# LMNS3d/SOFTX_2020_200

Hardware: AMD Instinct MI355X
Metric: nonlinear iters/sec (3D cavity Q2 128^3 BDF2) (higher is better)
Workload: dtype f64; 1 GPU; 3D lid-driven cavity Q2-Q2 128^3 transient BDF2 (BASELINE configs[2]); n_dofs=67898372, n_cells=2097152, parallelism=single

## Files before the change

include/gls_native.h:

```cpp
#ifndef GLS_NATIVE_H
#define GLS_NATIVE_H

#include <stddef.h>
#include <stdint.h>

#ifdef __cplusplus
extern "C" {
#endif

#define GLS_OK 0
#define GLS_EINVAL -1
#define GLS_EHIP -2
#define GLS_ENOMEM -3
#define GLS_ENOCONV -4
#define GLS_EIO -5
#define GLS_ECOMM -6
#define GLS_ENOTFOUND -7

enum gls_scheme {
  GLS_STEADY = 0, GLS_BDF1, GLS_BDF2, GLS_BDF3, GLS_SDIRK2, GLS_SDIRK2_1, GLS_SDIRK2_2,
  GLS_SDIRK3, GLS_SDIRK3_1, GLS_SDIRK3_2, GLS_SDIRK3_3
};

const char *gls_last_error(void);
// ... 76 lines not shown
  double coarse_omega;
  int coarse_direct;
  int mixed_precision;
  const int *level_sweeps;
  int smoother;
  int smoother_operator;
} gls_mg_params;
int gls_mg_attach(gls_ctx *ctx, const gls_mg_params *prm);
int gls_mg_attach_transfers(gls_ctx *ctx, const gls_mg_params *prm, const int64_t *const *p_off,
                            const int32_t *const *p_col, const double *const *p_w, const int64_t *const *inject);
int gls_mg_attach_replica(gls_ctx *ctx, const gls_mg_params *prm, gls_ctx *replica, const int64_t *p_off,
                          const int32_t *p_col, const double *p_w, const int64_t *inject);
int gls_apply_preconditioner(gls_ctx *ctx, const double *v, double *z);
int gls_mg_smoother_apply(gls_ctx *ctx, const double *v, double *y);
int gls_mg_transfer(gls_ctx *ctx, int level, int direction, const double *in, double *out);
int gls_set_lattice(gls_ctx *ctx, int n1d, const int64_t *local_to_global);
int gls_mg_detach(gls_ctx *ctx);
int gls_mg_set_coarse_replica(gls_ctx *ctx, gls_ctx *replica, int64_t n_local, const int64_t *local_to_replica);
#define GLS_ILU_MAX_FILL 10
int gls_ilu_attach(gls_ctx *ctx, int fill, double athresh, double rthresh);
int gls_ilu_detach(gls_ctx *ctx);
#define GLS_ILU_ORDER_CM 0
#define GLS_ILU_ORDER_MULTICOLOR 1
int gls_ilu_set_options(gls_ctx *ctx, int ordering, int64_t block_dofs);
int gls_ilu_info(const gls_ctx *ctx, int64_t *nnz, int *n_probes);
int gls_ilu_matrix(gls_ctx *ctx, int32_t *rowp, int32_t *col, double *val);
int gls_ilu_factors(gls_ctx *ctx, int32_t *perm, int32_t *rowp, int32_t *col, double *val);
int gls_iluk_pattern(int64_t n, const int32_t *rowp, const int32_t *col, int fill, int32_t *out_rowp,
                     int32_t *out_col, int32_t *out_level, int64_t capacity, int64_t *out_nnz);
int gls_cuthill_mckee(int64_t n_nodes, const int64_t *adj_off, const int64_t *adj, const int64_t *dof_off,
// ... 225 lines not shown
```

softx_2020_200_amd/csrc/gls_api.cpp:

```cpp
#include <hip/hip_runtime.h>

#include <algorithm>
#include <array>
#include <chrono>
#include <cmath>
#include <cstdlib>
#include <cstdarg>
#include <cstdio>
#include <cstring>
#include <map>
#include <array>
#include <memory>
#include <string>
#include <vector>
#include <set>
#include <thread>

#include <rocblas/rocblas.h>
#include <rocsolver/rocsolver.h>
#include <rocsparse/rocsparse.h>
#include <rccl/rccl.h>

#include "../../include/gls_native.h"
#include "gls_common.hpp"
// ... 387 lines not shown
    DevBuf<int32_t> map;
  } lat;
  struct MG {
    bool on = false;
    bool boxed = false;
    std::vector<gls_ctx *> lev;
    std::vector<std::array<int, 3>> dims;
    int k = 2, pre = 2, post = 2, csweeps = 30;
    std::vector<int> lpre, lpost;
    double omega = 0.6, comega = 0.6;
    std::vector<std::unique_ptr<DevBuf<double>>> bufs;
    struct Taps {
      DevBuf<int32_t> pi[3], ri[3], pc[3], rc[3];
      DevBuf<double> pw[3], rw[3];
      bool two_pass = false;
    };
    std::vector<std::unique_ptr<Taps>> taps;
    bool csr = false;
    bool ilu_smooth = false;
    struct Csr {
      DevBuf<int64_t> poff, roff;
      DevBuf<int32_t> pcol, rcol, inj;
      DevBuf<double> pw, rw;
      int64_t nf = 0, nc = 0;
      int plane = 1, rlane = 1;
    };
    std::vector<std::unique_ptr<Csr>> xfer;
    std::vector<gls_ctx *> ilu_levels;
    DevBuf<double> xwork;
    bool direct = false, direct_ok = false;
// ... 2124 lines not shown
    const auto &T = *mg.taps[(size_t)l];
    const int32_t *ti[3] = {T.pi[0].p, T.pi[1].p, T.pi[2].p}, *tc[3] = {T.pc[0].p, T.pc[1].p, T.pc[2].p};
    const double *tw[3] = {T.pw[0].p, T.pw[1].p, T.pw[2].p};
    if (T.two_pass)
      HIP_TRY(gls::mg_transfer_2pass(xb, mg_box_target(c, l, y), mg.dims[l + 1].data(), mg.dims[l].data(), 0, ti, tw,
                                     tc, mg.xwork.p, s, add ? 1 : 0));
    else if (add)
      return set_err(GLS_EINVAL, "mg_prolong: accumulate needs the two-pass transfer");
    else
      HIP_TRY(gls::mg_transfer3d(xb, mg_box_target(c, l, y), mg.dims[l + 1].data(), mg.dims[l].data(), ti, tw, tc, s));
  }
  GLS_TRY(mg_from_box(c, l, y));
  return GLS_OK;
}

bool coarse_graph_eligible(gls_ctx *c, gls_ctx *g, const double *b, const double *x) {
  const int l = (int)c->mg.lev.size() - 1;
  return !c->mg.cgraph_failed && !c->mg.boxed && !g->dist.on && !g->hang.on && g->use_brick && g->use_qdata &&
         brick_slab(g) && gls::brick_fused_jacobi_supported(g->k) && g->stream == c->stream &&
         b == mgbuf(c, l, MB_B) && x == mgbuf(c, l, MB_X) && std::getenv("GLS_MG_NO_FUSE") == nullptr &&
         std::getenv("GLS_MG_GRAPH") != nullptr;
}
}
static std::vector<unsigned char> coarse_graph_key(gls_ctx *g, const double *b, const double *x, const double *y,
                                                   int pre, double om) {
  const gls::OpParams P = make_params(g);
  const void *ptrs[7] = {b, x, y, g->diag.p, g->qdata.p, g->qdata32.p, brick_slab(g)};
  const int64_t ints[4] = {pre, g->n_dofs, (int64_t)g->smooth_f32, (int64_t)slab_f32()};
  std::vector<unsigned char> k(sizeof(P) + sizeof(ptrs) + sizeof(ints) + sizeof(om));
  unsigned char *o = k.data();
// ... 209 lines not shown
    }
  }
  const bool first_fused = pre == 1 && l < L - 1 && first_sweep_fusable(g);
  double *zs = mg.ilu_smooth && g->ilu.on && !g->ilu.probe_only ? mgbuf(c, l, MB_BOX) : nullptr;
  if (pre > 0 && !first_fused && zs) {
    GLS_TRY(ensure_ilu(g));
    GLS_TRY(apply_ilu(g, b, x));
    for (int it = 1; it < pre; ++it) GLS_TRY(smoother_sweep(g, x, b, y, om, zs));
  } else if (pre > 0 && !first_fused) {
    HIP_TRY(gls::mg_jacobi_update(x, b, nullptr, d, om, n, 1, s));
    for (int it = 1; it < pre; ++it) GLS_TRY(smoother_sweep(g, x, b, y, om));
  } else if (pre == 0) {
    HIP_TRY(gls::vec_fill(x, n, 0.0, s));
  }
  if (l == L - 1) return GLS_OK;
  if (first_fused) {
    GLS_TRY(jacobian_apply_f32(g, x, y, b, om, g->smooth_oseen));
  } else if (pre > 0) {
    GLS_TRY(smoother_apply(g, x, y, b));
  } else {
    HIP_TRY(gls::vec_copy(y, b, n, s));
  }
  gls_ctx *h = mg.lev[l + 1];
  double *bc = mgbuf(c, l + 1, MB_B), *xc = mgbuf(c, l + 1, MB_X);
  GLS_TRY(mg_restrict(c, l, y, bc));
  HIP_TRY(gls::vec_set_indexed(bc, h->con_dofs.p, nullptr, (int64_t)h->con_dofs.n, s));
  GLS_TRY(mg_vcycle(c, l + 1, bc, xc));
  if (mg_prolong_add_ok(c, l)) {
    GLS_TRY(mg_prolong(c, l, xc, x, true));
  } else {
    GLS_TRY(mg_prolong(c, l, xc, y));
    HIP_TRY(gls::vec_set_indexed(y, g->con_dofs.p, nullptr, (int64_t)g->con_dofs.n, s));
    HIP_TRY(gls::vec_axpy(x, 1.0, y, n, s));
  }
  for (int it = 0; it < mg.lpost[(size_t)l]; ++it) GLS_TRY(smoother_sweep(g, x, b, y, mg.omega, zs));
  return GLS_OK;
}

#define RS_TRY(x)                                                                        \
  do {                                                                                   \
    const rocsparse_status rs_ = (x);                                                    \
// ... 211 lines not shown
  if (c->mg.on) GLS_TRY(mg_prepare(c));
  GLS_TRY(ensure_ilu(c));
  return apply_prec(c, v, z);
}

int gls_mg_transfer(gls_ctx *c, int level, int direction, const double *in, double *out) {
  GLS_TRY(check_ctx(c));
  auto &mg = c->mg;
  if (!mg.on) return set_err(GLS_EINVAL, "gls_mg_transfer: no multigrid attached");
  if (level < 0 || level + 1 >= (int)mg.lev.size() || (direction != 0 && direction != 1) || !in || !out || in == out)
    return set_err(GLS_EINVAL, "gls_mg_transfer: bad level / direction / pointers");
  if (direction == 0) return mg_restrict(c, level, in, out);
  double *xc = mgbuf(c, level + 1, MB_X);
  HIP_TRY(gls::vec_copy(xc, in, mg.lev[(size_t)level + 1]->n_dofs, c->stream));
  return mg_prolong(c, level, xc, out);
}

namespace {
int build_face_neighbours(gls_ctx *c) {
  const int dim = c->dim, k = c->k, nv = gls::ipow(k + 1, dim);
  std::vector<int32_t> cn((size_t)c->n_cells * nv);
  if (!cn.empty() && hipMemcpy(cn.data(), c->cell_vnodes.p, cn.size() * sizeof(int32_t), hipMemcpyDeviceToHost) != hipSuccess)
    return set_err(GLS_EHIP, "cell map download failed");
  std::map<std::array<int32_t, 4>, std::pair<int, int>> open;
  std::vector<int32_t> nbr((size_t)c->n_cells * 2 * dim, -1);
  for (int cell = 0; cell < c->n_cells; ++cell)
    for (int d = 0; d < dim; ++d)
      for (int sd = 0; sd < 2; ++sd) {
        std::array<int32_t, 4> key = {-1, -1, -1, -1};
        int nk = 0;
// ... 353 lines not shown
      }
    } else {
      const int n = (int)std::lround(std::cbrt((double)g->n_vnodes));
      if ((int64_t)n * n * n != g->n_vnodes) return set_err(GLS_EINVAL, "mg level %d is not an n^3 lattice", l);
      if (l > 0 && mg.dims.back()[0] != 2 * n - 1) return set_err(GLS_EINVAL, "mg level %d not nested", l);
      dm = {n, n, n};
    }
    mg.lev.push_back(g);
    mg.dims.push_back(dm);
  }
  const int K = c->k;
  size_t xwork = 0;
  for (int l = 0; l + 1 < p->n_levels; ++l) {
    std::unique_ptr<gls_ctx::MG::Taps> T(new gls_ctx::MG::Taps);
    T->two_pass = true;
    xwork = std::max(xwork, (size_t)4 * mg.dims[l + 1][0] * mg.dims[l + 1][1] * mg.dims[l][2]);
    for (int a = 0; a < 3; ++a) {
      const int nf = mg.dims[l][a], nc = mg.dims[l + 1][a], ncc = (nf - 1) / (2 * K);
      std::vector<int32_t> pi((size_t)nf * 5, 0), ri((size_t)nc * 5, 0);
      std::vector<double> pw((size_t)nf * 5, 0.0), rw((size_t)nc * 5, 0.0);
      std::vector<int32_t> rn((size_t)nc, 0), pn((size_t)nf, 0);
      for (int i = 0; i < nf; ++i) {
        const double x = (double)i / (2.0 * K);
        const int cc = std::min((int)std::floor(x), ncc - 1);
        const double xi = x - cc;
        int np = 0;
        for (int q = 0; q <= K; ++q) {
          double L = 1.0;
          for (int b = 0; b <= K; ++b)
            if (b != q) L *= (xi * K - b) / (double)(q - b);
          if (L == 0.0) continue;
          const int j = cc * K + q;
          pi[(size_t)i * 5 + np] = j;
          pw[(size_t)i * 5 + np] = L;
          ++np;
          if (rn[(size_t)j] >= 5) return set_err(GLS_EINVAL, "mg: restriction stencil wider than 5");
          ri[(size_t)j * 5 + rn[(size_t)j]] = i;
          rw[(size_t)j * 5 + rn[(size_t)j]] = L;
          ++rn[(size_t)j];
        }
        pn[(size_t)i] = np;
      }
      if (a < 2)
        T->two_pass = T->two_pass && gls::mg_transfer_tile_fits(0, a, nf, pi.data(), pn.data()) &&
                      gls::mg_transfer_tile_fits(1, a, nc, ri.data(), rn.data());
      GLS_TRY(T->pi[a].upload(pi.data(), pi.size()));
      GLS_TRY(T->pw[a].upload(pw.data(), pw.size()));
      GLS_TRY(T->ri[a].upload(ri.data(), ri.size()));
      GLS_TRY(T->rw[a].upload(rw.data(), rw.size()));
      GLS_TRY(T->pc[a].upload(pn.data(), pn.size()));
      GLS_TRY(T->rc[a].upload(rn.data(), rn.size()));
    }
    mg.taps.push_back(std::move(T));
  }
  if (xwork) GLS_TRY(mg.xwork.alloc(xwork));
  return mg_attach_common(c, p);
// ... 1851 lines not shown
```

softx_2020_200_amd/csrc/gls_brick_kernels.hip:

```cpp
#include "gls_brick_common.hpp"
#include "gls_common.hpp"
#include "gls_launch.hpp"

#include <algorithm>
#include <cstdlib>
#include <type_traits>

#ifndef GLS_ABL
#define GLS_ABL 0
#endif
#ifndef GLS_ROWS_REG
#define GLS_ROWS_REG 1
#endif
#ifndef GLS_BRICK_WAVES_PER_EU
#define GLS_BRICK_WAVES_PER_EU 4
#endif
#ifndef GLS_BRICK_WPE_F32
#define GLS_BRICK_WPE_F32 6
#endif

#ifndef GLS_QD_LITE
#define GLS_QD_LITE 0
#endif

// ... 1206 lines not shown
    if (jb) hipLaunchKernelGGL((k_slab_sum_cube<float, true, KK>), g, b, 0, s, slabf, nb1, voff, y, vmask, jb, jd, jomega, rb, x0);  \
    else hipLaunchKernelGGL((k_slab_sum_cube<float, false, KK>), g, b, 0, s, slabf, nb1, voff, y, vmask, jb, jd, jomega, rb, x0);   \
  } else {                                                                                                                  \
    if (jb) hipLaunchKernelGGL((k_slab_sum_cube<double, true, KK>), g, b, 0, s, slab, nb1, voff, y, vmask, jb, jd, jomega, rb, x0); \
    else hipLaunchKernelGGL((k_slab_sum_cube<double, false, KK>), g, b, 0, s, slab, nb1, voff, y, vmask, jb, jd, jomega, rb, x0);  \
  }
  if (k == 1) {
    GLS_SLAB_CUBE(1)
  } else {
    GLS_SLAB_CUBE(2)
  }
#undef GLS_SLAB_CUBE
  return hipGetLastError();
}

bool brick_fused_jacobi_supported(int k) { return brick_impl(k) == 0 && (k == 1 || k == 2); }
#ifdef GLS_BRICK_COLORS_BUILD
bool brick_colors_supported(int k) { return brick_impl(k) == 0 && (k == 1 || k == 2); }
#else
bool brick_colors_supported(int) { return false; }
#endif
bool brick_subset_supported(int k) { return brick_impl(k) == 0 && (k == 1 || k == 2); }

size_t brick_qdata_size(int k, int n_cells) {
  if (brick_impl(k) == 1) return brick_wave_qdata_size(k, n_cells);
  return k == 1 ? brick_qdata_doubles<1>(n_cells) : (k == 2 ? brick_qdata_doubles<2>(n_cells) : 0);
}

hipError_t launch_brick_kernel(int k, int mode, const OpParams &P, const Tables1D &T, hipStream_t s) {
  if (mode == MODE_DIAG) return hipErrorNotSupported;
// ... 8 lines not shown
```

softx_2020_200_amd/csrc/gls_brick_pencil.hip:

```cpp
#include "gls_brick_common.hpp"
#include "gls_common.hpp"
#include "gls_launch.hpp"

#include <cstdlib>
#include <type_traits>

#ifndef GLS_PENCIL_WPE64
#define GLS_PENCIL_WPE64 2
#endif
#ifndef GLS_PENCIL_PIPE
#define GLS_PENCIL_PIPE 1
#endif
#ifndef GLS_PENCIL_NT
#define GLS_PENCIL_NT 0
#endif
#ifndef GLS_PENCIL_WPE32
#define GLS_PENCIL_WPE32 4
#endif

namespace gls {

template <typename Real, bool JV>
struct PencilCfg {
  static constexpr int K1 = 3, N3 = 27, BN = 5, BN3 = 125, BN3P = 128, NBND = 98;
// ... 17 lines not shown
  using C = PencilCfg<Real, JV>;
  return sizeof(Real) * ((size_t)C::BPG * pencil_fields(mode) * C::FB + (size_t)C::WAVES * C::CPW * C::CS +
                         (size_t)C::CPG * C::OC) +
         sizeof(int) * (size_t)C::BPG * C::BN3P;
}
template <typename Real>
size_t pencil_lds_bytes(int mode) {
  return mode == MODE_JVQ ? pencil_lds_bytes_t<Real, true>(mode) : pencil_lds_bytes_t<Real, false>(mode);
}

template <typename Real>
struct PencilTab {
  Real V[3][3], D[3][3], S[3][3], w[3], xi[3];
};

template <typename Real, int MODE, bool GEN, bool FOREST = false, bool OS = false>
__global__ void __launch_bounds__(256, (std::is_same<Real, float>::value ? GLS_PENCIL_WPE32 : GLS_PENCIL_WPE64))
    gls_pencil_kernel(const OpParams P, const PencilTab<Real> T) {
  static_assert(!OS || (MODE == MODE_JVQ && std::is_same<Real, float>::value), "Oseen operator: FP32 J.v only");
  using C = PencilCfg<Real, MODE == MODE_JVQ>;
  constexpr bool RL = MODE == MODE_RESLIN, RES = MODE == MODE_RESIDUAL || RL, LIN = MODE == MODE_LIN || RL;
  constexpr bool ST = RES || LIN;
  constexpr int BN = C::BN, BN3 = C::BN3, BN3P = C::BN3P, NF = pencil_fields(MODE);
  extern __shared__ __attribute__((aligned(16))) char smem_raw[];
  constexpr int FB = C::FB, SY = C::SY, SZ = C::SZ;
  Real *const sB = reinterpret_cast<Real *>(smem_raw);
  Real *const sS = sB + C::BPG * NF * FB;
  constexpr int CS = C::CS;
  Real *const sO = sS + C::WAVES * C::CPW * CS;
  int *const sNode = reinterpret_cast<int *>(sO + C::CPG * C::OC);
  __shared__ Real sRow[3 * 16];

  const int tid = threadIdx.x, lane = tid & 63, wave = tid >> 6;
  const int n_bricks = P.n_cells / 8;
// ... 249 lines not shown
          *reinterpret_cast<d2 *>(slo + si + 2) = d2{(double)s[2], (double)s[3]};
        }
      }
    }
  };

  auto write_ev = [&]() {
    for (int t = tid; t < nbg * 8 * 27; t += C::THREADS) {
      const int rb_ = t / 216, r = t - rb_ * 216, ci_ = r / 27, a = r - ci_ * 27;
      const Real *o = sO + (rb_ * 8 + ci_) * C::OC + a;
      double *e = P.ev + (cell0(brick_of(rb_)) + ci_) * 108;
      e[a * 3] = (double)o[0];
      e[a * 3 + 1] = (double)o[C::OF];
      e[a * 3 + 2] = (double)o[2 * C::OF];
      e[81 + a] = (double)o[3 * C::OF];
    }
  };

  if constexpr (ST) {
    Real uq[3][3], Ttq[3][3], pq[3], gp[3][3];
    {
      Real dz[3];
#pragma unroll
      for (int cc = 0; cc < 3; ++cc) {
        Real bb[3], hb[3];
        forward(cc, 0, bb, dz, dz, dz);
        forward(4 + cc, 0, hb, dz, dz, dz);
#pragma unroll
        for (int qz = 0; qz < 3; ++qz) {
          uq[cc][qz] = zval(bb, qz);
// ... 298 lines not shown
      const Real JxW = wxy * T.w[qz], jt = JxW * tauq[qz];
      const Real Tv = JxW * divv[qz];
      const Real Tx = jt * Sq[0][qz] * ihx, Ty = jt * Sq[1][qz] * ihy, Tz = jt * Sq[2][qz] * ihz;
#pragma unroll
      for (int az = 0; az < 3; ++az) {
        Z[0][az] += T.V[qz][az] * Tv + T.D[qz][az] * Tz;
        Z[1][az] += T.V[qz][az] * Tx;
        Z[2][az] += T.V[qz][az] * Ty;
      }
    }
    backward(3, Z);
  }
  }
  __syncthreads();

  if (P.ev) write_ev();
  else reduce_scatter(P.y, P.slab, true);
}


bool pencil_enabled() {
  const char *e = std::getenv("GLS_PENCIL");
  return !(e && std::atoi(e) == 0);
}

template <typename Real, int MODE, bool FB = false>
hipError_t launch_pencil_t(const OpParams &P, const Tables1D &T, hipStream_t s) {
  const bool gen = P.srf || (MODE != MODE_JVQ && P.force_q);
  const int n_items = ((std::is_same<Real, double>::value || P.brick_cell0) && P.subset) ? P.subset_n : P.n_cells / 8;
  if (n_items <= 0) return hipSuccess;
  const int n_groups = (n_items + 2) / 3;
  PencilTab<Real> tab;
// ... 18 lines not shown
    }
  }
  if (gen)
    hipLaunchKernelGGL((gls_pencil_kernel<Real, MODE, true, FB>), dim3((unsigned)n_groups), dim3(256),
                       pencil_lds_bytes<Real>(MODE), s, P, tab);
  else
    hipLaunchKernelGGL((gls_pencil_kernel<Real, MODE, false, FB>), dim3((unsigned)n_groups), dim3(256),
                       pencil_lds_bytes<Real>(MODE), s, P, tab);
  return hipGetLastError();
}
hipError_t launch_pencil_jv(const OpParams &P, const Tables1D &T, hipStream_t s, bool f32) {
  if (P.n_probe > 0 || P.bricks || !(f32 ? (P.slabf != nullptr || P.slab != nullptr) : P.slab != nullptr))
    return hipErrorNotSupported;
  return f32 ? launch_pencil_t<float, MODE_JVQ>(P, T, s) : launch_pencil_t<double, MODE_JVQ>(P, T, s);
}
hipError_t launch_pencil_residual(const OpParams &P, const Tables1D &T, hipStream_t s) {
  if (P.bricks || !P.slab || P.subset) return hipErrorNotSupported;
  return launch_pencil_t<double, MODE_RESIDUAL>(P, T, s);
}
hipError_t launch_pencil_reslin(const OpParams &P, const Tables1D &T, hipStream_t s) {
  if (P.bricks || P.subset || !P.qd || !P.y || !P.slab || !P.res_y || !P.res_slab) return hipErrorNotSupported;
  return launch_pencil_t<double, MODE_RESLIN>(P, T, s);
}
hipError_t launch_pencil_ev(int mode, const OpParams &P, const Tables1D &T, hipStream_t s, bool f32) {
  if ((!P.ev && mode != MODE_LIN) || P.y || !P.brick_cell0 || !P.subset || P.subset_n <= 0 || !P.qd || P.slab ||
      P.bricks || P.n_probe > 0 || P.rb || P.jx || P.jx0 || (f32 && (mode != MODE_JVQ || !P.qdf)))
    return hipErrorNotSupported;
  if (mode == MODE_JVQ && f32) return launch_pencil_t<float, MODE_JVQ, true>(P, T, s);
  if (mode == MODE_JVQ) return launch_pencil_t<double, MODE_JVQ>(P, T, s);
  if (mode == MODE_LIN) return launch_pencil_t<double, MODE_LIN>(P, T, s);
// ... 9 lines not shown
```

softx_2020_200_amd/csrc/gls_common.hpp:

```cpp
#pragma once
#include <hip/hip_runtime.h>

#include <cstdint>

namespace gls {

constexpr int kMaxNodes1D = 4;
constexpr int kMaxQ1D = 5;

constexpr int ipow(int b, int e) { return e == 0 ? 1 : b * ipow(b, e - 1); }

enum Mode { MODE_RESIDUAL = 0, MODE_JV = 1, MODE_DIAG = 2, MODE_LIN = 3, MODE_JVQ = 4,
            MODE_RESLIN = 5  };
constexpr int kQData = 16;

struct Tables1D {
  double V[kMaxQ1D][kMaxNodes1D];
  double D[kMaxQ1D][kMaxNodes1D];
  double S[kMaxQ1D][kMaxNodes1D];
  double Vp[kMaxQ1D][kMaxNodes1D];
  double Dp[kMaxQ1D][kMaxNodes1D];
  double w[kMaxQ1D];
  double xi[kMaxQ1D];
};
// ... 45 lines not shown
  const int32_t *bricks;
  const uint16_t *ncolor;
  double *acc;
  int n_colors;
  int color;
  int color_off[17];
  double nu;
  double alpha[4];
  double alpha_jac;
  double sdt2;
  int srf;
  double omega[3];
  int oseen;
  double *cq;
  int cq_mode;
};

}
```

softx_2020_200_amd/csrc/gls_launch.hpp:

```cpp
#pragma once
#include "gls_common.hpp"

namespace gls {

hipError_t gather_element_vectors(double *y, const double *ev, const int64_t *voff, const int64_t *vslot, int64_t nv,
                                  const int64_t *poff, const int64_t *pslot, int64_t np, int dim, hipStream_t s);
hipError_t launch_cell_kernel(int dim, int k, int kp, int nq1d, int mode, const OpParams &P, const Tables1D &T,
                              hipStream_t s);
bool cell_kernel_supported(int dim, int k, int kp, int nq1d);
hipError_t launch_cell_sf_jv(int dim, int k, int kp, int nq1d, const OpParams &P, const Tables1D &T, hipStream_t s);
bool cell_sf_enabled();
int cell_kernel_cells_per_block(int dim, int k, int nq1d, bool probe = false);
hipError_t launch_brick_kernel(int k, int mode, const OpParams &P, const Tables1D &T, hipStream_t s);
size_t brick_qdata_size(int k, int n_cells);
hipError_t launch_brick_jv_f32(int k, const OpParams &P, const Tables1D &T, hipStream_t s);
hipError_t vec_to_f32(const double *a, float *b, int64_t n, hipStream_t s);
hipError_t vec_from_f32(const float *a, double *b, int64_t n, hipStream_t s);
hipError_t launch_pencil_jv(const OpParams &P, const Tables1D &T, hipStream_t s, bool f32);
hipError_t launch_pencil_residual(const OpParams &P, const Tables1D &T, hipStream_t s);
hipError_t launch_pencil_lin(const OpParams &P, const Tables1D &T, hipStream_t s);
hipError_t launch_pencil_reslin(const OpParams &P, const Tables1D &T, hipStream_t s);
hipError_t launch_pencil_ev(int mode, const OpParams &P, const Tables1D &T, hipStream_t s, bool f32 = false);
bool pencil_enabled();
hipError_t launch_brick_wave(int k, int mode, const OpParams &P, const Tables1D &T, hipStream_t s);
hipError_t launch_brick_wave_jv_f32(int k, const OpParams &P, const Tables1D &T, hipStream_t s);
hipError_t launch_brick_wave_probe(int k, const OpParams &P, const Tables1D &T, int64_t j0, int nprobe, hipStream_t s);
size_t brick_wave_qdata_size(int k, int n_cells);

int brick_boundary_nodes(int k);
hipError_t brick_slab_sum(const double *slab, const int32_t *nodes, const int32_t *off, const int32_t *slots,
                          int64_t n_sum, int64_t n_vnodes, double *y, hipStream_t s);
hipError_t brick_slab_sum_ex(const double *slab, const float *slabf, const int32_t *nodes, const int32_t *off,
                             const int32_t *slots, int64_t n_sum, int64_t n_vnodes, double *y, const uint8_t *vmask,
                             const double *jb, const double *jd, double jomega, hipStream_t s,
                             const double *rb = nullptr);
hipError_t brick_slab_sum_cube(int k, int nb1, const double *slab, const float *slabf, int64_t n_vnodes, double *y,
                               const uint8_t *vmask, const double *jb, const double *jd, double jomega, hipStream_t s,
                               const double *rb = nullptr, double *x0 = nullptr);
bool brick_fused_jacobi_supported(int k);
bool brick_colors_supported(int k);
bool brick_subset_supported(int k);
hipError_t launch_brick_probe(int k, const OpParams &P, const Tables1D &T, int64_t j0, int nprobe, hipStream_t s);

hipError_t vec_fill(double *x, int64_t n, double a, hipStream_t s);
hipError_t vec_copy(double *y, const double *x, int64_t n, hipStream_t s);
hipError_t vec_axpy(double *y, double a, const double *x, int64_t n, hipStream_t s);
hipError_t vec_axpby(double *y, double a, const double *x, double b, int64_t n, hipStream_t s);
hipError_t vec_scale(double *x, double a, int64_t n, hipStream_t s);
hipError_t vec_div(double *y, const double *x, const double *d, int64_t n, hipStream_t s);
hipError_t vec_multidot(const double *A, int64_t lda, int nk, const double *w, int64_t n, double *out,
                        double *work, hipStream_t s);
hipError_t vec_multidot2(const double *A, int64_t lda, int nk, const double *w, int64_t n1, int64_t off2, int64_t n2,
                         double *out, double *work, hipStream_t s);
// ... 117 lines not shown
```

softx_2020_200_amd/native.py:

```python
from __future__ import annotations

import ctypes as C
import os

import numpy as np

HERE = os.path.dirname(os.path.abspath(__file__))
LIB_PATH = os.environ.get("GLS_NATIVE_LIB") or os.path.join(HERE, "libgls_native.so")

GLS_OK, GLS_EINVAL, GLS_EHIP, GLS_ENOMEM, GLS_ENOCONV, GLS_EIO, GLS_ECOMM = 0, -1, -2, -3, -4, -5, -6

SCHEMES = {
    "steady": 0, "bdf1": 1, "bdf2": 2, "bdf3": 3, "sdirk2": 4, "sdirk2_1": 5, "sdirk2_2": 6,
    "sdirk3": 7, "sdirk3_1": 8, "sdirk3_2": 9, "sdirk3_3": 10,
}

EXPORTS = [
    "gls_last_error", "gls_version", "gls_create", "gls_destroy", "gls_set_stream", "gls_n_dofs", "gls_set_force",
    "gls_set_viscosity", "gls_set_time", "gls_set_state", "gls_residual", "gls_jacobian_apply",
    "gls_jacobian_apply_f32",
    "gls_jacobian_diagonal", "gls_set_dirichlet", "gls_apply_dirichlet", "gls_solve_linear", "gls_newton_solve",
    "gls_bdf_coefficients", "gls_sdirk_coefficients", "gls_newton_selftest", "gls_mesh_hyper_cube_sizes",
    "gls_mesh_hyper_cube", "gls_timing_reset", "gls_timing_get", "gls_timing_enable", "gls_uses_brick_kernels",
    "gls_part_create", "gls_part_sizes", "gls_part_get", "gls_part_destroy", "gls_dist_attach", "gls_dist_import", "gls_rccl_unique_id", "gls_rccl_create", "gls_rccl_destroy", "gls_rccl_info", "gls_mg_smoother_apply", "gls_mg_attach_replica",
    "gls_dist_attach_rccl",
    "gls_mg_attach", "gls_mg_detach", "gls_mg_set_coarse_replica", "gls_residual_and_diagonal", "gls_octree_set_periodic", "gls_ilu_attach", "gls_ilu_detach", "gls_ilu_info", "gls_ilu_matrix", "gls_ilu_factors", "gls_ilu_set_options", "gls_iluk_pattern", "gls_cuthill_mckee", "gls_section_timing", "gls_section_get", "gls_dist_attach_dofs", "gls_dist_attach_dofs_rccl", "gls_gpart_create", "gls_gpart_sizes", "gls_gpart_get", "gls_gpart_map_dofs", "gls_gpart_destroy", "gls_dpart_create", "gls_set_lattice", "gls_apply_preconditioner", "gls_mg_transfer",
    "gls_prm_parse", "gls_prm_get", "gls_prm_n_entries", "gls_prm_entry", "gls_prm_destroy",
    "gls_expr_create", "gls_expr_n_components", "gls_expr_eval", "gls_expr_destroy",
    "gls_vtu_write", "gls_pvtu_write", "gls_pvd_write",
    "gls_set_hanging", "gls_mesh_refined_create", "gls_mesh_refined_destroy", "gls_octree_create", "gls_octree_destroy", "gls_octree_info",
    "gls_octree_cells", "gls_octree_adapt", "gls_octree_prepare", "gls_octree_mesh", "gls_octree_mesh_destroy", "gls_octree_transfer", "gls_octree_faces", "gls_kelly_estimate_faces",
    "gls_kelly_estimate", "gls_refine_fixed_number", "gls_mesh_refined_interpolate", "gls_refine_pd", "gls_refine_coarsen_pd",
    "gls_freeze_jacobian", "gls_skip_newton_selftest", "gls_quadrature_points",
    "gls_umesh_generate", "gls_umesh_read_gmsh", "gls_umesh_set_manifold", "gls_umesh_boundary_manifold",
    "gls_umesh_refine_global", "gls_umesh_info", "gls_umesh_destroy", "gls_umesh_fe_space", "gls_fe_space_destroy",
    "gls_fe_space_transfer", "gls_umesh_prepare", "gls_umesh_adapt", "gls_umesh_set_periodic", "gls_fe_space_kelly_faces",
    "gls_kelly_estimate_mapped", "gls_fe_space_boundary_normals", "gls_fe_space_boundary_normal_sets",
    "gls_octree_coarsen_to", "gls_octree_mg_transfer", "gls_mg_attach_transfers", "gls_umesh_coarsen_to",
    "gls_fe_space_mg_transfer", "gls_forest_bricks",
    "gls_fe_space_boundary_faces", "gls_boundary_plan_create", "gls_boundary_plan_destroy", "gls_boundary_loads",
]
# ... 119 lines not shown
    L.gls_mg_set_coarse_replica.argtypes = [vp, vp, i64, C.POINTER(i64)]
    L.gls_mg_attach_transfers.argtypes = [vp, C.POINTER(MGParams), C.POINTER(C.POINTER(i64)),
                                          C.POINTER(C.POINTER(C.c_int32)), C.POINTER(C.POINTER(C.c_double)),
                                          C.POINTER(C.POINTER(i64))]
    L.gls_octree_coarsen_to.argtypes = [vp, C.c_int, C.POINTER(vp)]
    L.gls_umesh_coarsen_to.argtypes = [vp, C.c_int, C.POINTER(vp)]
    L.gls_forest_bricks.argtypes = [vp]
    L.gls_fe_space_mg_transfer.argtypes = [C.POINTER(FESpace), C.POINTER(FESpace), C.POINTER(i64), vp, vp, vp, vp]
    L.gls_octree_mg_transfer.argtypes = [C.POINTER(RefinedMesh), C.POINTER(RefinedMesh), C.POINTER(i64), vp, vp, vp, vp]
    L.gls_set_lattice.argtypes = [vp, C.c_int, C.POINTER(i64)]
    L.gls_apply_preconditioner.argtypes = [vp, vp, vp]
    L.gls_mg_smoother_apply.argtypes = [vp, vp, vp]
    L.gls_mg_attach_replica.argtypes = [vp, C.POINTER(MGParams), vp, C.POINTER(C.c_int64), C.POINTER(C.c_int32),
                                        C.POINTER(C.c_double), C.POINTER(C.c_int64)]
    L.gls_mg_transfer.argtypes = [vp, C.c_int, C.c_int, vp, vp]
    P64 = C.POINTER(i64)
    L.gls_set_hanging.argtypes = [vp, i64, P64, P64, P64, d]
    L.gls_mesh_refined_create.argtypes = [C.c_int, C.c_int, C.c_int, C.c_int, C.c_double, C.c_double,
                                          C.POINTER(C.c_int32), C.POINTER(C.POINTER(RefinedMesh))]
    L.gls_mesh_refined_destroy.argtypes = [C.POINTER(RefinedMesh)]
    L.gls_kelly_estimate.argtypes = [vp, vp, C.c_int, vp]
    L.gls_refine_fixed_number.argtypes = [i64, C.POINTER(C.c_float), C.c_double, C.POINTER(C.c_int32)]
    L.gls_refine_pd.argtypes = [i64, C.POINTER(C.c_float), C.c_int, C.c_int, C.c_double, i64,
                                C.POINTER(C.c_int32), C.POINTER(C.c_double)]
    L.gls_mesh_refined_interpolate.argtypes = [C.POINTER(RefinedMesh), C.c_int, C.c_double, C.c_double,
                                               C.POINTER(C.c_double), C.POINTER(C.c_double)]
    L.gls_quadrature_points.argtypes = [vp, d]
    L.gls_umesh_generate.argtypes = [C.c_int, C.c_char_p, C.c_char_p, C.POINTER(vp)]
    L.gls_umesh_read_gmsh.argtypes = [C.c_int, C.c_char_p, C.POINTER(vp)]
    L.gls_umesh_set_manifold.argtypes = [vp, C.c_int, C.c_int, d, d]
# ... 612 lines not shown
        check(self.L.gls_boundary_plan_create(self.h, len(sl), int(faces["nqf"]), p32(f["cell"]), p32(sl), _dp(f["xi"]),
                                              _dp(f["jinv"]), _dp(f["normal"]), _dp(f["jxw"]), _dp(f["xq"]),
                                              int(n_slots), C.byref(plan)), "gls_boundary_plan_create")
        force, torque = np.zeros((int(n_slots), 3)), np.zeros((int(n_slots), 3))
        try:
            check(self.L.gls_boundary_loads(self.h, plan, _ptr(sol), float(viscosity), _dp(cor), _dp(force), _dp(torque)),
                  "gls_boundary_loads")
        finally:
            self.L.gls_boundary_plan_destroy(plan)
        return force, torque

    def mg_transfer(self, level, direction, v, out):
        check(self.L.gls_mg_transfer(self.h, int(level), int(direction), _ptr(v), _ptr(out)), "gls_mg_transfer")
        return out

    def set_lattice(self, n1d, local_to_global):
        l2g = np.ascontiguousarray(local_to_global, dtype=np.int64)
        check(self.L.gls_set_lattice(self.h, int(n1d), l2g.ctypes.data_as(C.POINTER(C.c_int64))), "gls_set_lattice")

    def detach_multigrid(self):
        check(self.L.gls_mg_detach(self.h), "gls_mg_detach")
        self._mg_levels = None

    def attach_ilu(self, athresh=1e-8, rthresh=1.0, fill=0, block_dofs=0, ordering="cm"):
        self.L.gls_ilu_set_options.argtypes = [C.c_void_p, C.c_int, C.c_int64]
        check(self.L.gls_ilu_set_options(self.h, {"cm": 0, "multicolor": 1}[ordering], int(block_dofs)),
              "gls_ilu_set_options")
        self.L.gls_ilu_attach.argtypes = [C.c_void_p, C.c_int, C.c_double, C.c_double]
        check(self.L.gls_ilu_attach(self.h, int(fill), float(athresh), float(rthresh)), "gls_ilu_attach")
        nnz, npr = C.c_int64(), C.c_int()
# ... 268 lines not shown
```

Baseline: 11.51 nonlinear_iters/s.

## Fuse multigrid residual computation with Q2 restriction inside the pencil operator kernel

Adds a restriction epilogue to the FP32 pencil J.v kernel. It computes the residual b - Av per brick in LDS, applies the 5-to-3 Q2 restriction stencil along each axis, and writes per-brick coarse contributions to the slab. A new cube-sum kernel then gathers these into the coarse right-hand side and applies Dirichlet masking. This replaces the separate smoother-apply, two-pass transfer and constrained-dof zeroing kernels, with the aim of cutting full fine-level vector round trips in each V-cycle. It only applies under many eligibility conditions (structured cube, Q2 weights, brick/slab path), and it adds LDS pressure and new code paths.

```diff
diff --git a/include/gls_native.h b/include/gls_native.h
--- a/include/gls_native.h
+++ b/include/gls_native.h
@@ -114,6 +114,7 @@
 int gls_apply_preconditioner(gls_ctx *ctx, const double *v, double *z);
 int gls_mg_smoother_apply(gls_ctx *ctx, const double *v, double *y);
 int gls_mg_transfer(gls_ctx *ctx, int level, int direction, const double *in, double *out);
+int gls_mg_residual_restrict(gls_ctx *ctx, int level, const double *x, const double *b, double *bc, int *fused);
 int gls_set_lattice(gls_ctx *ctx, int n1d, const int64_t *local_to_global);
 int gls_mg_detach(gls_ctx *ctx);
 int gls_mg_set_coarse_replica(gls_ctx *ctx, gls_ctx *replica, int64_t n_local, const int64_t *local_to_replica);
diff --git a/softx_2020_200_amd/csrc/gls_api.cpp b/softx_2020_200_amd/csrc/gls_api.cpp
--- a/softx_2020_200_amd/csrc/gls_api.cpp
+++ b/softx_2020_200_amd/csrc/gls_api.cpp
@@ -425,6 +425,7 @@
       DevBuf<int32_t> pi[3], ri[3], pc[3], rc[3];
       DevBuf<double> pw[3], rw[3];
       bool two_pass = false;
+      bool q2_brick = false;
     };
     std::vector<std::unique_ptr<Taps>> taps;
     bool csr = false;
@@ -2579,6 +2580,46 @@
   return GLS_OK;
 }
 
+bool mg_fused_restrict_ok(gls_ctx *c, int l) {
+  auto &mg = c->mg;
+  if (l < 0 || l + 1 >= (int)mg.lev.size() || mg.csr || mg.boxed || (size_t)l >= mg.taps.size()) return false;
+  const char *e = std::getenv("GLS_MG_FUSE_TRANSFER");
+  if ((e && std::atoi(e) == 0) || std::getenv("GLS_MG_NO_FUSE") != nullptr) return false;
+  gls_ctx *g = mg.lev[(size_t)l], *h = mg.lev[(size_t)l + 1];
+  const auto &T = *mg.taps[(size_t)l];
+  const int64_t nc1 = 2 * (int64_t)g->cube_nb1 + 1;
+  return T.two_pass && T.q2_brick && g->smooth_f32 && g->use_brick && g->use_qdata && !g->use_colors && !g->dist.on &&
+         !g->hang.on && !g->oct.on && g->k == 2 && g->cube_nb1 > 0 && g->cube_nb1 < 1024 && g->use_slab && !g->srf &&
+         gls::pencil_enabled() && gls::brick_fused_jacobi_supported(g->k) && !h->dist.on && !h->hang.on &&
+         h->n_vnodes == nc1 * nc1 * nc1 && g->stream == c->stream;
+}
+int mg_residual_restrict_fused(gls_ctx *c, int l, double *x, const double *b, double *bc, double first_omega = 0.0) {
+  gls_ctx *g = c->mg.lev[(size_t)l], *h = c->mg.lev[(size_t)l + 1];
+  if (!g->u) return set_err(GLS_EINVAL, "gls_set_state was not called");
+  GLS_TRY(ensure_diag(g));
+  GLS_TRY(ensure_qdata32(g, !g->smooth_oseen));
+  gls::OpParams P = make_params(g, true);
+  P.qdf = g->qdata32.p;
+  P.oseen = g->smooth_oseen ? 1 : 0;
+  P.v = x;
+  P.rb = b;
+  P.cube_nb1 = g->cube_nb1;
+  if (first_omega > 0.0) {
+    P.jx0 = x;
+    P.jd = g->diag.p;
+    P.jomega = first_omega;
+  }
+  P.slab = brick_slab(g);
+  if (!P.slab) return set_err(GLS_EHIP, "brick slab allocation failed");
+  {
+    TimedLaunch t(g, 4);
+    HIP_TRY(gls::launch_pencil_jv_restrict(P, g->tables, c->stream));
+  }
+  TimedLaunch t(g, 5);
+  HIP_TRY(gls::brick_restrict_sum_cube(g->cube_nb1, P.slab, h->n_vnodes, bc, h->vmask.p, c->stream));
+  return GLS_OK;
+}
+
 bool coarse_graph_eligible(gls_ctx *c, gls_ctx *g, const double *b, const double *x) {
   const int l = (int)c->mg.lev.size() - 1;
   return !c->mg.cgraph_failed && !c->mg.boxed && !g->dist.on && !g->hang.on && g->use_brick && g->use_qdata &&
@@ -2818,17 +2859,21 @@
     HIP_TRY(gls::vec_fill(x, n, 0.0, s));
   }
   if (l == L - 1) return GLS_OK;
-  if (first_fused) {
-    GLS_TRY(jacobian_apply_f32(g, x, y, b, om, g->smooth_oseen));
-  } else if (pre > 0) {
-    GLS_TRY(smoother_apply(g, x, y, b));
-  } else {
-    HIP_TRY(gls::vec_copy(y, b, n, s));
-  }
   gls_ctx *h = mg.lev[l + 1];
   double *bc = mgbuf(c, l + 1, MB_B), *xc = mgbuf(c, l + 1, MB_X);
-  GLS_TRY(mg_restrict(c, l, y, bc));
-  HIP_TRY(gls::vec_set_indexed(bc, h->con_dofs.p, nullptr, (int64_t)h->con_dofs.n, s));
+  if (pre > 0 && mg_fused_restrict_ok(c, l)) {
+    GLS_TRY(mg_residual_restrict_fused(c, l, x, b, bc, first_fused ? om : 0.0));
+  } else {
+    if (first_fused) {
+      GLS_TRY(jacobian_apply_f32(g, x, y, b, om, g->smooth_oseen));
+    } else if (pre > 0) {
+      GLS_TRY(smoother_apply(g, x, y, b));
+    } else {
+      HIP_TRY(gls::vec_copy(y, b, n, s));
+    }
+    GLS_TRY(mg_restrict(c, l, y, bc));
+    HIP_TRY(gls::vec_set_indexed(bc, h->con_dofs.p, nullptr, (int64_t)h->con_dofs.n, s));
+  }
   GLS_TRY(mg_vcycle(c, l + 1, bc, xc));
   if (mg_prolong_add_ok(c, l)) {
     GLS_TRY(mg_prolong(c, l, xc, x, true));
@@ -3070,6 +3115,24 @@
   double *xc = mgbuf(c, level + 1, MB_X);
   HIP_TRY(gls::vec_copy(xc, in, mg.lev[(size_t)level + 1]->n_dofs, c->stream));
   return mg_prolong(c, level, xc, out);
+}
+
+int gls_mg_residual_restrict(gls_ctx *c, int level, const double *x, const double *b, double *bc, int *fused) {
+  GLS_TRY(check_ctx(c));
+  auto &mg = c->mg;
+  if (!mg.on) return set_err(GLS_EINVAL, "gls_mg_residual_restrict: no multigrid attached");
+  if (level < 0 || level + 1 >= (int)mg.lev.size() || !x || !b || !bc)
+    return set_err(GLS_EINVAL, "gls_mg_residual_restrict: bad level / pointers");
+  GLS_TRY(mg_prepare(c));
+  const bool f = mg_fused_restrict_ok(c, level);
+  if (fused) *fused = f ? 1 : 0;
+  if (f) return mg_residual_restrict_fused(c, level, const_cast<double *>(x), b, bc);
+  gls_ctx *g = mg.lev[(size_t)level], *h = mg.lev[(size_t)level + 1];
+  double *y = mgbuf(c, level, MB_Y);
+  GLS_TRY(smoother_apply(g, x, y, b));
+  GLS_TRY(mg_restrict(c, level, y, bc));
+  HIP_TRY(gls::vec_set_indexed(bc, h->con_dofs.p, nullptr, (int64_t)h->con_dofs.n, c->stream));
+  return GLS_OK;
 }
 
 namespace {
@@ -3453,7 +3516,8 @@
   for (int l = 0; l + 1 < p->n_levels; ++l) {
     std::unique_ptr<gls_ctx::MG::Taps> T(new gls_ctx::MG::Taps);
     T->two_pass = true;
-    xwork = std::max(xwork, (size_t)4 * mg.dims[l + 1][0] * mg.dims[l + 1][1] * mg.dims[l][2]);
+    T->q2_brick = K == 2;
+    xwork =std::max(xwork, (size_t)4 * mg.dims[l + 1][0] * mg.dims[l + 1][1] * mg.dims[l][2]);
     for (int a = 0; a < 3; ++a) {
       const int nf = mg.dims[l][a], nc = mg.dims[l + 1][a], ncc = (nf - 1) / (2 * K);
       std::vector<int32_t> pi((size_t)nf * 5, 0), ri((size_t)nc * 5, 0);
@@ -3479,6 +3543,18 @@
           ++rn[(size_t)j];
         }
         pn[(size_t)i] = np;
+        if (K == 2) {
+          static const double W[5][3] = {{1, 0, 0}, {0.375, 0.75, -0.125}, {0, 1, 0}, {-0.125, 0.75, 0.375}, {0, 0, 1}};
+          const int m = i - 4 * cc;
+          int nz = 0;
+          for (int q = 0; q < 3; ++q) nz += W[m][q] != 0.0;
+          bool same = np == nz;
+          for (int e = 0; same && e < np; ++e) {
+            const int q = pi[(size_t)i * 5 + e] - 2 * cc;
+            same = q >= 0 && q < 3 && pw[(size_t)i * 5 + e] == W[m][q];
+          }
+          T->q2_brick = T->q2_brick && same && nf == 2 * nc - 1;
+        }
       }
       if (a < 2)
         T->two_pass = T->two_pass && gls::mg_transfer_tile_fits(0, a, nf, pi.data(), pn.data()) &&
diff --git a/softx_2020_200_amd/csrc/gls_brick_kernels.hip b/softx_2020_200_amd/csrc/gls_brick_kernels.hip
--- a/softx_2020_200_amd/csrc/gls_brick_kernels.hip
+++ b/softx_2020_200_amd/csrc/gls_brick_kernels.hip
@@ -1244,6 +1244,91 @@
   return hipGetLastError();
 }
 
+__global__ void __launch_bounds__(256) k_restrict_sum_cube(const double *__restrict__ ev, int nb1, int64_t voff,
+                                                           double *__restrict__ bc, const uint8_t *__restrict__ vmask) {
+  const int NX = 2 * nb1 + 1;
+  int bx = blockIdx.x, Z = blockIdx.y;
+  if (GLS_SLAB_XCD) {
+    const int lin = xcd_swizzle((int)(blockIdx.x + gridDim.x * blockIdx.y), (int)(gridDim.x * gridDim.y));
+    bx = lin % (int)gridDim.x;
+    Z = lin / (int)gridDim.x;
+  }
+  const int64_t t = (int64_t)bx * blockDim.x + threadIdx.x;
+  if (t >= (int64_t)NX * NX) return;
+  const int X = (int)(t % NX), Y = (int)(t / NX);
+  int bcd[3][2], lc[3][2], nc[3];
+  const int co[3] = {X, Y, Z};
+#pragma unroll
+  for (int d = 0; d < 3; ++d) {
+    const int x = co[d];
+    if (x % 2 == 0 && x > 0 && x < NX - 1) {
+      nc[d] = 2;
+      bcd[d][0] = x / 2 - 1;
+      lc[d][0] = 2;
+      bcd[d][1] = x / 2;
+      lc[d][1] = 0;
+    } else {
+      nc[d] = 1;
+      bcd[d][0] = min(x / 2, nb1 - 1);
+      lc[d][0] = x - 2 * bcd[d][0];
+      bcd[d][1] = bcd[d][0];
+      lc[d][1] = lc[d][0];
+    }
+  }
+  int64_t sl[8];
+  int cnt = 0;
+#pragma unroll
+  for (int k = 0; k < 2; ++k)
+#pragma unroll
+    for (int j = 0; j < 2; ++j)
+#pragma unroll
+      for (int i = 0; i < 2; ++i) {
+        const bool on = i < nc[0] && j < nc[1] && k < nc[2];
+        const int64_t s = (int64_t)morton3(bcd[0][i], bcd[1][j], bcd[2][k]) * 27 + lc[0][i] + 3 * (lc[1][j] + 3 * lc[2][k]);
+        sl[i + 2 * j + 4 * k] = on ? s : INT64_MAX;
+        cnt += on;
+      }
+  auto cs = [&](int a, int b) {
+    const int64_t lo = min(sl[a], sl[b]), hi = max(sl[a], sl[b]);
+    sl[a] = lo;
+    sl[b] = hi;
+  };
+  cs(0, 1); cs(2, 3); cs(4, 5); cs(6, 7);
+  cs(0, 2); cs(1, 3); cs(4, 6); cs(5, 7);
+  cs(1, 2); cs(5, 6); cs(0, 4); cs(3, 7);
+  cs(1, 5); cs(2, 6);
+  cs(1, 4); cs(3, 6);
+  cs(2, 4); cs(3, 5);
+  cs(3, 4);
+  double e[8][4];
+#pragma unroll
+  for (int q = 0; q < 8; ++q)
+    if (q < cnt) SlabQuad<double>::load(ev + sl[q] * 4, e[q][0], e[q][1], e[q][2], e[q][3]);
+  double s[4] = {0., 0., 0., 0.};
+#pragma unroll
+  for (int q = 0; q < 8; ++q)
+    if (q < cnt) {
+      s[0] += e[q][0];
+      s[1] += e[q][1];
+      s[2] += e[q][2];
+      s[3] += e[q][3];
+    }
+  const int64_t node = X + (int64_t)NX * (Y + (int64_t)NX * Z);
+  const unsigned m = vmask ? vmask[node] : 0u;
+  bc[node * 3] = (m & 1u) ? 0.0 : s[0];
+  bc[node * 3 + 1] = (m & 2u) ? 0.0 : s[1];
+  bc[node * 3 + 2] = (m & 4u) ? 0.0 : s[2];
+  bc[voff + node] = s[3];
+}
+hipError_t brick_restrict_sum_cube(int nb1, const double *ev, int64_t n_vnodes, double *bc, const uint8_t *vmask,
+                                   hipStream_t s) {
+  const int64_t NX = 2 * (int64_t)nb1 + 1;
+  if (nb1 <= 0 || nb1 > 1023 || !ev || !bc || NX * NX * NX != n_vnodes) return hipErrorInvalidValue;
+  const dim3 g((unsigned)((NX * NX + 255) / 256), (unsigned)NX), b(256);
+  hipLaunchKernelGGL(k_restrict_sum_cube, g, b, 0, s, ev, nb1, 3 * n_vnodes, bc, vmask);
+  return hipGetLastError();
+}
+
 bool brick_fused_jacobi_supported(int k) { return brick_impl(k) == 0 && (k == 1 || k == 2); }
 #ifdef GLS_BRICK_COLORS_BUILD
 bool brick_colors_supported(int k) { return brick_impl(k) == 0 && (k == 1 || k == 2); }
diff --git a/softx_2020_200_amd/csrc/gls_brick_pencil.hip b/softx_2020_200_amd/csrc/gls_brick_pencil.hip
--- a/softx_2020_200_amd/csrc/gls_brick_pencil.hip
+++ b/softx_2020_200_amd/csrc/gls_brick_pencil.hip
@@ -55,10 +55,11 @@
   Real V[3][3], D[3][3], S[3][3], w[3], xi[3];
 };
 
-template <typename Real, int MODE, bool GEN, bool FOREST = false, bool OS = false>
+template <typename Real, int MODE, bool GEN, bool FOREST = false, bool OS = false, bool RST = false>
 __global__ void __launch_bounds__(256, (std::is_same<Real, float>::value ? GLS_PENCIL_WPE32 : GLS_PENCIL_WPE64))
     gls_pencil_kernel(const OpParams P, const PencilTab<Real> T) {
   static_assert(!OS || (MODE == MODE_JVQ && std::is_same<Real, float>::value), "Oseen operator: FP32 J.v only");
+  static_assert(!RST || (MODE == MODE_JVQ && std::is_same<Real, float>::value && !FOREST), "restriction: FP32 J.v on the cube");
   using C = PencilCfg<Real, MODE == MODE_JVQ>;
   constexpr bool RL = MODE == MODE_RESLIN, RES = MODE == MODE_RESIDUAL || RL, LIN = MODE == MODE_LIN || RL;
   constexpr bool ST = RES || LIN;
@@ -338,6 +339,98 @@
       e[a * 3 + 1] = (double)o[C::OF];
       e[a * 3 + 2] = (double)o[2 * C::OF];
       e[81 + a] = (double)o[3 * C::OF];
+    }
+  };
+
+  auto restrict_store = [&]() {
+    auto r53 = [](double r0, double r1, double r2, double r3, double r4, double &c0, double &c1, double &c2) {
+      c0 = r0 + (0.375 * r1 - 0.125 * r3);
+      c1 = r2 + 0.75 * (r1 + r3);
+      c2 = r4 + (0.375 * r3 - 0.125 * r1);
+    };
+    auto compact3 = [](unsigned v) {
+      v &= 0x09249249u;
+      v = (v ^ (v >> 2)) & 0x030c30c3u;
+      v = (v ^ (v >> 4)) & 0x0300f00fu;
+      v = (v ^ (v >> 8)) & 0xff0000ffu;
+      return (int)((v ^ (v >> 16)) & 0x3ffu);
+    };
+    static_assert((C::BPG * NF * FB + C::WAVES * C::CPW * CS) % 2 == 0 && C::BPG * NF * FB + C::WAVES * C::CPW * CS >= 2 * (C::BPG * 4 * (BN3 + 45)) &&
+                      C::CPG * C::OC >= 2 * C::BPG * 4 * 75, "restriction scratch in LDS");
+    double *const dR = reinterpret_cast<double *>(sB), *const dY = dR + C::BPG * 4 * BN3;
+    double *const dX = reinterpret_cast<double *>(sO);
+    for (int t = tid; t < C::BPG * BN3; t += C::THREADS) {
+      const int rb_ = t / BN3, n = t % BN3;
+      if (rb_ >= nbg) break;
+      const int bk = brick_of(rb_);
+      const int Xn = n % BN, Yn = (n / BN) % BN, Zn = n / (BN * BN);
+      Real s[4] = {0, 0, 0, 0};
+#pragma unroll
+      for (int kz = 0; kz < 2; ++kz) {
+        const int az = Zn - 2 * kz;
+        if (az < 0 || az > 2) continue;
+#pragma unroll
+        for (int ky = 0; ky < 2; ++ky) {
+          const int ay = Yn - 2 * ky;
+          if (ay < 0 || ay > 2) continue;
+#pragma unroll
+          for (int kx = 0; kx < 2; ++kx) {
+            const int ax = Xn - 2 * kx;
+            if (ax < 0 || ax > 2) continue;
+            const Real *o = sO + (rb_ * 8 + kx + 2 * ky + 4 * kz) * C::OC + ax + 3 * (ay + 3 * az);
+#pragma unroll
+            for (int f = 0; f < 4; ++f) s[f] += o[f * C::OF];
+          }
+        }
+      }
+      const int node = sNode[rb_ * BN3P + n];
+      const int top = P.cube_nb1 - 1;
+      const bool own = (Xn < BN - 1 || compact3((unsigned)bk) == top) && (Yn < BN - 1 || compact3((unsigned)bk >> 1) == top) &&
+                       (Zn < BN - 1 || compact3((unsigned)bk >> 2) == top);
+      const unsigned m = P.vmask ? P.vmask[node] : 0u;
+      double r[4] = {-(double)s[0], -(double)s[1], -(double)s[2], -(double)s[3]};
+      if (own) {
+        const int64_t gi[4] = {(int64_t)node * 3, (int64_t)node * 3 + 1, (int64_t)node * 3 + 2, voff + node};
+#pragma unroll
+        for (int f = 0; f < 4; ++f) r[f] = P.rb[gi[f]] - (double)s[f];
+        if (P.jx0) {
+#pragma unroll
+          for (int f = 0; f < 4; ++f) P.jx0[gi[f]] = 0.0 + P.jomega * P.rb[gi[f]] / P.jd[gi[f]];
+        }
+      }
+#pragma unroll
+      for (int f = 0; f < 4; ++f) dR[(rb_ * 4 + f) * BN3 + n] = (f < 3 && ((m >> f) & 1u)) ? 0.0 : r[f];
+    }
+    __syncthreads();
+    for (int t = tid; t < nbg * 4 * 25; t += C::THREADS) {
+      const int bf = t / 25, yz = t - bf * 25;
+      const double *r = dR + bf * BN3 + BN * yz;
+      double *o = dX + bf * 75 + 3 * yz;
+      r53(r[0], r[1], r[2], r[3], r[4], o[0], o[1], o[2]);
+    }
+    __syncthreads();
+    for (int t = tid; t < nbg * 4 * 15; t += C::THREADS) {
+      const int bf = t / 15, zx = t - bf * 15, Z = zx / 3, cx_ = zx - 3 * Z;
+      const double *r = dX + bf * 75 + 15 * Z + cx_;
+      double *o = dY + bf * 45 + 9 * Z + cx_;
+      r53(r[0], r[3], r[6], r[9], r[12], o[0], o[3], o[6]);
+    }
+    __syncthreads();
+    for (int t = tid; t < nbg * 9; t += C::THREADS) {
+      const int rb_ = t / 9, xy = t - rb_ * 9;
+      double cv[4][3];
+#pragma unroll
+      for (int f = 0; f < 4; ++f) {
+        const double *r = dY + (rb_ * 4 + f) * 45 + xy;
+        r53(r[0], r[9], r[18], r[27], r[36], cv[f][0], cv[f][1], cv[f][2]);
+      }
+      typedef double d2 __attribute__((ext_vector_type(2)));
+      d2 *e = reinterpret_cast<d2 *>(P.slab + ((int64_t)brick_of(rb_) * 27 + xy) * 4);
+#pragma unroll
+      for (int cz_ = 0; cz_ < 3; ++cz_) {
+        e[18 * cz_] = d2{cv[0][cz_], cv[1][cz_]};
+        e[18 * cz_ + 1] = d2{cv[2][cz_], cv[3][cz_]};
+      }
     }
   };
 
@@ -666,8 +759,12 @@
   }
   __syncthreads();
 
-  if (P.ev) write_ev();
-  else reduce_scatter(P.y, P.slab, true);
+  if constexpr (RST) {
+    restrict_store();
+  } else {
+    if (P.ev) write_ev();
+    else reduce_scatter(P.y, P.slab, true);
+  }
 }
 
 
@@ -716,6 +813,29 @@
     return hipErrorNotSupported;
   return f32 ? launch_pencil_t<float, MODE_JVQ>(P, T, s) : launch_pencil_t<double, MODE_JVQ>(P, T, s);
 }
+hipError_t launch_pencil_jv_restrict(const OpParams &P, const Tables1D &T, hipStream_t s) {
+  if (P.n_probe > 0 || P.bricks || P.subset || P.brick_cell0 || P.srf || !P.slab || !P.rb || !P.qdf || P.jx || (P.jx0 && !P.jd) ||
+      P.cube_nb1 <= 0 || (int64_t)P.cube_nb1 * P.cube_nb1 * P.cube_nb1 * 8 != P.n_cells)
+    return hipErrorNotSupported;
+  const int n_groups = (P.n_cells / 8 + 2) / 3;
+  PencilTab<float> tab;
+  for (int q = 0; q < 3; ++q) {
+    tab.w[q] = (float)T.w[q];
+    for (int i = 0; i < 3; ++i) {
+      tab.V[q][i] = (float)T.V[q][i];
+      tab.D[q][i] = (float)T.D[q][i];
+      tab.S[q][i] = (float)T.S[q][i];
+    }
+    tab.xi[q] = (float)T.xi[q];
+  }
+  if (P.oseen)
+    hipLaunchKernelGGL((gls_pencil_kernel<float, MODE_JVQ, false, false, true, true>), dim3((unsigned)n_groups), dim3(256),
+                       pencil_lds_bytes<float>(MODE_JVQ), s, P, tab);
+  else
+    hipLaunchKernelGGL((gls_pencil_kernel<float, MODE_JVQ, false, false, false, true>), dim3((unsigned)n_groups), dim3(256),
+                       pencil_lds_bytes<float>(MODE_JVQ), s, P, tab);
+  return hipGetLastError();
+}
 hipError_t launch_pencil_residual(const OpParams &P, const Tables1D &T, hipStream_t s) {
   if (P.bricks || !P.slab || P.subset) return hipErrorNotSupported;
   return launch_pencil_t<double, MODE_RESIDUAL>(P, T, s);
diff --git a/softx_2020_200_amd/csrc/gls_common.hpp b/softx_2020_200_amd/csrc/gls_common.hpp
--- a/softx_2020_200_amd/csrc/gls_common.hpp
+++ b/softx_2020_200_amd/csrc/gls_common.hpp
@@ -83,6 +83,7 @@
   int oseen;
   double *cq;
   int cq_mode;
+  int cube_nb1;
 };
 
 }
diff --git a/softx_2020_200_amd/csrc/gls_launch.hpp b/softx_2020_200_amd/csrc/gls_launch.hpp
--- a/softx_2020_200_amd/csrc/gls_launch.hpp
+++ b/softx_2020_200_amd/csrc/gls_launch.hpp
@@ -17,6 +17,7 @@
 hipError_t vec_to_f32(const double *a, float *b, int64_t n, hipStream_t s);
 hipError_t vec_from_f32(const float *a, double *b, int64_t n, hipStream_t s);
 hipError_t launch_pencil_jv(const OpParams &P, const Tables1D &T, hipStream_t s, bool f32);
+hipError_t launch_pencil_jv_restrict(const OpParams &P, const Tables1D &T, hipStream_t s);
 hipError_t launch_pencil_residual(const OpParams &P, const Tables1D &T, hipStream_t s);
 hipError_t launch_pencil_lin(const OpParams &P, const Tables1D &T, hipStream_t s);
 hipError_t launch_pencil_reslin(const OpParams &P, const Tables1D &T, hipStream_t s);
@@ -37,6 +38,8 @@
 hipError_t brick_slab_sum_cube(int k, int nb1, const double *slab, const float *slabf, int64_t n_vnodes, double *y,
                                const uint8_t *vmask, const double *jb, const double *jd, double jomega, hipStream_t s,
                                const double *rb = nullptr, double *x0 = nullptr);
+hipError_t brick_restrict_sum_cube(int nb1, const double *ev, int64_t n_vnodes, double *bc, const uint8_t *vmask,
+                                   hipStream_t s);
 bool brick_fused_jacobi_supported(int k);
 bool brick_colors_supported(int k);
 bool brick_subset_supported(int k);
diff --git a/softx_2020_200_amd/native.py b/softx_2020_200_amd/native.py
--- a/softx_2020_200_amd/native.py
+++ b/softx_2020_200_amd/native.py
@@ -25,6 +25,7 @@
     "gls_part_create", "gls_part_sizes", "gls_part_get", "gls_part_destroy", "gls_dist_attach", "gls_dist_import", "gls_rccl_unique_id", "gls_rccl_create", "gls_rccl_destroy", "gls_rccl_info", "gls_mg_smoother_apply", "gls_mg_attach_replica",
     "gls_dist_attach_rccl",
     "gls_mg_attach", "gls_mg_detach", "gls_mg_set_coarse_replica", "gls_residual_and_diagonal", "gls_octree_set_periodic", "gls_ilu_attach", "gls_ilu_detach", "gls_ilu_info", "gls_ilu_matrix", "gls_ilu_factors", "gls_ilu_set_options", "gls_iluk_pattern", "gls_cuthill_mckee", "gls_section_timing", "gls_section_get", "gls_dist_attach_dofs", "gls_dist_attach_dofs_rccl", "gls_gpart_create", "gls_gpart_sizes", "gls_gpart_get", "gls_gpart_map_dofs", "gls_gpart_destroy", "gls_dpart_create", "gls_set_lattice", "gls_apply_preconditioner", "gls_mg_transfer",
+    "gls_mg_residual_restrict",
     "gls_prm_parse", "gls_prm_get", "gls_prm_n_entries", "gls_prm_entry", "gls_prm_destroy",
     "gls_expr_create", "gls_expr_n_components", "gls_expr_eval", "gls_expr_destroy",
     "gls_vtu_write", "gls_pvtu_write", "gls_pvd_write",
@@ -174,6 +175,7 @@
     L.gls_mg_attach_replica.argtypes = [vp, C.POINTER(MGParams), vp, C.POINTER(C.c_int64), C.POINTER(C.c_int32),
                                         C.POINTER(C.c_double), C.POINTER(C.c_int64)]
     L.gls_mg_transfer.argtypes = [vp, C.c_int, C.c_int, vp, vp]
+    L.gls_mg_residual_restrict.argtypes = [vp, C.c_int, vp, vp, vp, C.POINTER(C.c_int)]
     P64 = C.POINTER(i64)
     L.gls_set_hanging.argtypes = [vp, i64, P64, P64, P64, d]
     L.gls_mesh_refined_create.argtypes = [C.c_int, C.c_int, C.c_int, C.c_int, C.c_double, C.c_double,
@@ -816,6 +818,12 @@
         check(self.L.gls_mg_transfer(self.h, int(level), int(direction), _ptr(v), _ptr(out)), "gls_mg_transfer")
         return out
 
+    def mg_residual_restrict(self, level, x, b, out):
+        fused = C.c_int(0)
+        check(self.L.gls_mg_residual_restrict(self.h, int(level), _ptr(x), _ptr(b), _ptr(out), C.byref(fused)),
+              "gls_mg_residual_restrict")
+        return out, bool(fused.value)
+
     def set_lattice(self, n1d, local_to_global):
         l2g = np.ascontiguousarray(local_to_global, dtype=np.int64)
         check(self.L.gls_set_lattice(self.h, int(n1d), l2g.ctypes.data_as(C.POINTER(C.c_int64))), "gls_set_lattice")
```

New measurement: 12.42 nonlinear_iters/s, median of 6. 7.9% higher.
